# esologic/GANce

Measured on AMD Instinct MI355X. Metric: synthesized frames/sec at 1024x1024 config-f, higher is better.
Workload: dtype f32 (bf16x3 split operands, 6 terms, fp32 accumulate)

## Files before the change

### gance_amd/csrc/upfir_split.hip

```cpp

#include <hip/hip_runtime.h>

#include <algorithm>
#include <cstring>
#include <type_traits>

#include "kernels.h"

#ifndef GANCE_UPFIRS_ABLATE
#define GANCE_UPFIRS_ABLATE 0
#endif

namespace gance {

namespace {

typedef float f32x4 __attribute__((ext_vector_type(4)));
typedef float f32x2 __attribute__((ext_vector_type(2)));
typedef unsigned u32x4 __attribute__((ext_vector_type(4)));
typedef unsigned u32x2 __attribute__((ext_vector_type(2)));
typedef __bf16 bf16x8 __attribute__((ext_vector_type(8)));
typedef __bf16 bf16x2 __attribute__((ext_vector_type(2)));
typedef __attribute__((address_space(3))) void* lds_ptr_t;

constexpr int kBM = 16;
constexpr int kKC = 32;
constexpr int kSW = 64;
constexpr int kTH = 8;
constexpr int kRows = kTH + 1;
constexpr int kPlanes = 12;
constexpr int kPlaneStride = 80;
constexpr int kSlotUnits = kPlanes * kPlaneStride;
constexpr int kRing = 3;
constexpr int kHaloCols = 4;
constexpr int kHaloUnits = kRows * kHaloCols * kPlanes;
constexpr int kHaloTasks = kRows * kHaloCols * 4;
constexpr int kWeave = 2;
constexpr int kMinSegRows = 16;
constexpr int kDepth = 6;
constexpr int kCarryRows = 3;
constexpr int kPassCh = 4;
constexpr int kPassRows = 8;
constexpr float kSqrt2f = 1.4142135623730951f;
static_assert((2 * kRows) % kDepth == 0 && kDepth + 2 < kRows && kRows % kRing == 0, "ring slots and staging registers rotate with the unrolled rows of a chunk pair");

template <int NT>
struct Geo {
    static constexpr int kSW = 64 / NT;
    static constexpr int kBMB = kBM * NT;
    static constexpr int kTC = kSW / 16;
    static constexpr int kPW = 4 / NT;
    static constexpr int kTW = 2 * kSW + 4;
    static constexpr int kCG = kSW / 2;
    static constexpr int kRG = 64 / NT / kCG;
    static constexpr int kFR = kPassRows / kRG;
    static constexpr int kWin = kFR + 3;
    static constexpr int kCarryFloats = kBMB * kCarryRows * kTW;
    static constexpr int kStageFloats = kPassCh * NT * kPassRows * kTW;
    static constexpr int kNzPieces = 2 * kPassRows * 2 * kSW / 256;
    static constexpr int kWUnits = NT == 1 ? 27 * 64 : 0;
};

constexpr size_t kRingBytes = (size_t)kRing * kSlotUnits * 16;
constexpr size_t kHaloBytes = (size_t)2 * kHaloUnits * 16;
template <int NT>
constexpr size_t lds_bytes(int cin) {
    using G = Geo<NT>;
    return kRingBytes + kHaloBytes + (size_t)G::kWUnits * 16 +
           sizeof(float) * ((size_t)G::kStageFloats + G::kNzPieces * 256 + G::kCarryFloats + cin + 3 * G::kBMB);
}

__host__ __device__ constexpr int tap_cls(int t) { return t < 4 ? 0 : (t < 6 ? 1 : (t < 8 ? 2 : 3)); }
__host__ __device__ constexpr int tap_dy(int t) { return (t == 2 || t == 3 || t == 5) ? 1 : 0; }
__host__ __device__ constexpr int tap_dx(int t) { return (t == 1 || t == 3 || t == 7) ? 1 : 0; }

__device__ __forceinline__ void lds_barrier() {
    asm volatile("s_waitcnt lgkmcnt(0)" ::: "memory");
    __builtin_amdgcn_s_barrier();
    asm volatile("" ::: "memory");
}

__device__ __forceinline__ int fresh_lane() {
    int l;
    asm volatile("v_mbcnt_lo_u32_b32 %0, -1, 0\n\tv_mbcnt_hi_u32_b32 %0, -1, %0" : "=v"(l));
    return l;
}

__device__ __forceinline__ int ring_column(int P) {
    return ((P >> 2) & 3) | ((((P >> 4) ^ P) & 1) << 2) | (((P >> 1) & 1) << 3) | ((P & 1) << 4) | (P & 32);
}
constexpr int kEdgeColumn = 64;

__device__ __forceinline__ void split_pair(float a, float b, unsigned& p0, unsigned& p1, unsigned& p2) {
    auto pack = [](float lo, float hi) { return __builtin_bit_cast(unsigned, __builtin_convertvector(f32x2{lo, hi}, bf16x2)); };
    p0 = pack(a, b);
    const float ra = a - __builtin_bit_cast(float, p0 << 16), rb = b - __builtin_bit_cast(float, p0 & 0xffff0000u);
    p1 = pack(ra, rb);
    const float sa = ra - __builtin_bit_cast(float, p1 << 16), sb = rb - __builtin_bit_cast(float, p1 & 0xffff0000u);
    p2 = pack(sa, sb);
}

__device__ __forceinline__ void split_unit(const unsigned (&raw)[8], u32x4 (&part)[3]) {
    unsigned w[3][4];
    if (GANCE_UPFIRS_ABLATE & 1) {
#pragma unroll
        for (int q = 0; q < 3; ++q) part[q] = u32x4{raw[q], raw[q + 1], raw[q + 2], raw[q + 3]};
        return;
    }
#pragma unroll
    for (int e = 0; e < 4; ++e) split_pair(__builtin_bit_cast(float, raw[2 * e]), __builtin_bit_cast(float, raw[2 * e + 1]), w[0][e], w[1][e], w[2][e]);
#pragma unroll
    for (int q = 0; q < 3; ++q) part[q] = u32x4{w[q][0], w[q][1], w[q][2], w[q][3]};
}

}

template <int NT, bool kPre, bool kNoise>
__device__ __forceinline__ void upfirs_body(const UpFirArgs& p) {
    using G = Geo<NT>;
    constexpr int kSW = G::kSW, kBMB = G::kBMB, kTC = G::kTC, kPW = G::kPW, kTW = G::kTW, kCG = G::kCG, kRG = G::kRG, kFR = G::kFR,
                  kWin = G::kWin, kCarryFloats = G::kCarryFloats, kStageFloats = G::kStageFloats, kNzPieces = G::kNzPieces;
    extern __shared__ __attribute__((aligned(16))) unsigned char smem_raw[];
    u32x4* const ring = reinterpret_cast<u32x4*>(smem_raw);
    u32x4* const halo = ring + kRing * kSlotUnits;
    u32x4* const w_lds = halo + 2 * kHaloUnits;
    float* const stage = reinterpret_cast<float*>(w_lds + G::kWUnits);
    float* const nz_lds = stage + kStageFloats;
    float* const carry = nz_lds + kNzPieces * 256;
    float* const s_lds = carry + kCarryFloats;
    float* const d_lds = s_lds + (kPre ? 0 : p.Cin);
    float* const b_lds = d_lds + kBMB;
    float* const sn_lds = b_lds + kBMB;

    const int tid = threadIdx.x;
    const int wave = __builtin_amdgcn_readfirstlane(tid >> 6);
    const int lane = tid & 63;
    const int n16 = lane & 15, kg = lane >> 4;
    const int ct = NT == 1 ? 0 : wave / kTC, tc = NT == 1 ? wave : wave % kTC;

    int id;
    {
        const int v = blockIdx.x, nwg = p.total_blocks;
        const int q = nwg >> 3, r = nwg & 7, xcd = v & 7;
        id = (xcd < r ? xcd * (q + 1) : r * (q + 1) + (xcd - r) * q) + (v >> 3);
    }
    const int m_tile = id % p.m_tiles;
    id /= p.m_tiles;
    const int strip = id % p.strips;
    id /= p.strips;
    const int seg = id % p.segs;
    const int b = id / p.segs;
    const int m0 = m_tile * kBMB;
    const int X0 = strip * kSW;
    const int H = p.H, W = p.W;
    const int Hp = H + 2, Wp = W + 8;
    const int HpWp4 = Hp * Wp * 4;
    const int chunks = p.Cin / kKC;
    const int steps = H / kTH;
    const int s_begin = seg * (p.rows_per_seg / kTH), s_end = s_begin + p.rows_per_seg / kTH;
    const int s_first = seg > 0 ? s_begin - 1 : s_begin;

    const __amdgpu_buffer_rsrc_t x_rsrc =
        __builtin_amdgcn_make_buffer_rsrc((void*)(p.x + (size_t)b * p.x_b_stride), 0, p.Cin * Hp * Wp * 4, 0x00020000);
    const __amdgpu_buffer_rsrc_t w_rsrc = __builtin_amdgcn_make_buffer_rsrc(
        (void*)(reinterpret_cast<const unsigned char*>(p.w) + (size_t)(m_tile * NT + ct) * chunks * 27 * 1024), 0, chunks * 27 * 1024, 0x00020000);

    const int st_pair = lane >> 4, st_g = lane & 15;
    u32x4* const ring_w = ring + wave * kPlaneStride + ring_column(4 * st_g + st_pair);
    unsigned* const ring_wn = reinterpret_cast<unsigned*>(ring + wave * kPlaneStride + ring_column(NT == 2 ? 2 * st_g + (st_pair & 1) : st_g)) +
                              (NT == 2 ? 2 * (st_pair >> 1) : st_pair);
    const int m_pos = 16 * tc + n16;
    const u32x4* const ring_r0 = ring + kg * kPlaneStride + ring_column(m_pos);
    const u32x4* const ring_r1 = ring + kg * kPlaneStride + (m_pos > 0 ? ring_column(m_pos - 1) : kEdgeColumn);
    const bool edge_copy = wave == 3 && lane < kPlanes;
    const int e_unit = lane % kPlanes;
    u32x4* const ring_e = ring + (e_unit >> 2) * 4 * kPlaneStride + (e_unit & 3) * kPlaneStride + (edge_copy ? kEdgeColumn : 66 + wave);
    const u32x4* const halo_e = halo + e_unit;
    const u32x4* const halo_r = halo + ((n16 & 7) * kHaloCols + 2 * (n16 >> 3)) * kPlanes + kg;
    const u32x4* const halo_f = halo + ((kRows - 1) * kHaloCols + 2 * (n16 >> 3)) * kPlanes + kg;
    const int st_voff = (2 * st_pair * Hp * Wp + X0 + 4 + kPW * st_g) * 4;
    unsigned st[kDepth][8];
    auto stage_load = [&](unsigned(&dst)[8], int chunk, int brow, bool in_loop = false) {
        if ((GANCE_UPFIRS_ABLATE & 4) && in_loop) return;
        const int soff = ((chunk * kKC + wave * 8) * Hp + brow) * Wp * 4;
#pragma unroll
        for (int e = 0; e < 2; ++e) {
            if constexpr (kPW == 4) {
                const u32x4 q4 = __builtin_amdgcn_raw_buffer_load_b128(x_rsrc, st_voff, soff + e * HpWp4, 0);
#pragma unroll
                for (int c = 0; c < 4; ++c) dst[2 * c + e] = q4[c];
            } else if constexpr (kPW == 2) {
                const u32x2 q2 = __builtin_amdgcn_raw_buffer_load_b64(x_rsrc, st_voff, soff + e * HpWp4, 0);
                dst[e] = q2[0];
                dst[2 + e] = q2[1];
            } else {
                dst[e] = __builtin_amdgcn_raw_buffer_load_b32(x_rsrc, st_voff, soff + e * HpWp4, 0);
            }
        }
    };
    auto scale_pair = [&](unsigned(&raw)[8], int chunk) {
        if constexpr (!kPre) {
            const f32x2 s2 = *reinterpret_cast<const f32x2*>(s_lds + chunk * kKC + 8 * wave + 2 * st_pair);
#pragma unroll
            for (int c = 0; c < kPW; ++c) {
                raw[2 * c] = __builtin_bit_cast(unsigned, __builtin_bit_cast(float, raw[2 * c]) * s2[0]);
                raw[2 * c + 1] = __builtin_bit_cast(unsigned, __builtin_bit_cast(float, raw[2 * c + 1]) * s2[1]);
            }
        }
    };
    auto transpose_rows = [](u32x4& u) {
        auto a02 = __builtin_amdgcn_permlane32_swap(u[0], u[2], false, false);
        auto a13 = __builtin_amdgcn_permlane32_swap(u[1], u[3], false, false);
        auto b01 = __builtin_amdgcn_permlane16_swap(a02[0], a13[0], false, false);
        auto b23 = __builtin_amdgcn_permlane16_swap(a02[1], a13[1], false, false);
        u = u32x4{b01[0], b01[1], b23[0], b23[1]};
    };
    auto scale8 = [&](unsigned(&raw)[8], int chunk, int group) {
        if constexpr (!kPre) {
            const f32x4 s0 = *reinterpret_cast<const f32x4*>(s_lds + chunk * kKC + group * 8);
            const f32x4 s1 = *reinterpret_cast<const f32x4*>(s_lds + chunk * kKC + group * 8 + 4);
#pragma unroll
            for (int e = 0; e < 4; ++e) {
                raw[e] = __builtin_bit_cast(unsigned, __builtin_bit_cast(float, raw[e]) * s0[e]);
                raw[4 + e] = __builtin_bit_cast(unsigned, __builtin_bit_cast(float, raw[4 + e]) * s1[e]);
            }
        }
    };
    auto stage_store = [&](unsigned(&raw)[8], int slot, int chunk) {
        scale_pair(raw, chunk);
        if constexpr (NT == 1) {
            u32x4 part[3];
            split_unit(raw, part);
#pragma unroll
            for (int q = 0; q < 3; ++q) transpose_rows(part[q]);
#pragma unroll
            for (int q = 0; q < 3; ++q)
                if (!(GANCE_UPFIRS_ABLATE & 16)) ring_w[slot * kSlotUnits + q * 4 * kPlaneStride] = part[q];
        } else {
            unsigned w[3][kPW];
#pragma unroll
            for (int c = 0; c < kPW; ++c) split_pair(__builtin_bit_cast(float, raw[2 * c]), __builtin_bit_cast(float, raw[2 * c + 1]), w[0][c], w[1][c], w[2][c]);
#pragma unroll
            for (int q = 0; q < 3; ++q) {
                unsigned* const dst = ring_wn + 4 * (slot * kSlotUnits + q * 4 * kPlaneStride);
                if constexpr (NT == 2) {
                    const auto s = __builtin_amdgcn_permlane16_swap(w[q][0], w[q][1], false, false);
                    *reinterpret_cast<u32x2*>(dst) = u32x2{s[0], s[1]};
                } else {
                    *dst = w[q][0];
                }
            }
        }
    };
    auto edge_store = [&](int slot, int hbuf, int hrow) { if (!(GANCE_UPFIRS_ABLATE & 64)) ring_e[slot * kSlotUnits] = halo_e[hbuf * kHaloUnits + (hrow * kHaloCols + 1) * kPlanes]; };
    const int h_task = tid < kHaloTasks ? tid : tid - kHaloTasks;
    const int h_col = h_task & 3, h_kg = (h_task >> 2) & 3, h_row = h_task >> 4;
    const int h_voff = ((h_kg * 8 * Hp + h_row) * Wp + X0 + 2 + (h_col & 1) + (h_col >> 1) * (kSW + 1)) * 4;
    u32x4* const halo_w = halo + (h_row * kHaloCols + h_col) * kPlanes + h_kg;
    unsigned hraw[8];
    auto halo_load = [&](int step, int chunk) {
        const int soff = (chunk * kKC * Hp + kTH * step) * Wp * 4;
#pragma unroll
        for (int e = 0; e < 8; ++e) hraw[e] = __builtin_amdgcn_raw_buffer_load_b32(x_rsrc, h_voff, soff + e * HpWp4, 0);
    };
    auto halo_store = [&](int chunk, int buf) {
        scale8(hraw, chunk, h_kg);
        u32x4 part[3];
        split_unit(hraw, part);
#pragma unroll
        for (int q = 0; q < 3; ++q) halo_w[buf * kHaloUnits + q * 4] = part[q];
    };

    u32x4 A[9][3];
    const int a_voff = lane * 16;
    auto weights_dma = [&](int chunk) {
#pragma unroll
        for (int k = 0; k < 7; ++k)
            if (k < 6 || wave < 3)
                __builtin_amdgcn_raw_ptr_buffer_load_lds(w_rsrc, (lds_ptr_t)(w_lds + (wave + 4 * k) * 64), 16, lane * 16, (chunk * 27 + wave + 4 * k) * 1024, 0, 0);
    };
    const u32x4* const w_r = w_lds + lane;
    auto read_a3 = [&](int t, u32x4(&dst)[3]) {
#pragma unroll
        for (int q = 0; q < 3; ++q) dst[q] = w_r[(t * 3 + q) * 64];
    };
    auto load_a3 = [&](int chunk, int t, u32x4(&dst)[3]) {
#pragma unroll
        for (int q = 0; q < 3; ++q) dst[q] = __builtin_amdgcn_raw_buffer_load_b128(w_rsrc, a_voff, (chunk * 27 + t * 3 + q) * 1024, 0);
    };

    u32x4 Bf[2][2][3];
    auto load_b = [&](int slot, u32x4(&dst)[2][3]) {
#pragma unroll
        for (int q = 0; q < 3; ++q) {
            dst[0][q] = ring_r0[slot * kSlotUnits + q * 4 * kPlaneStride];
            dst[1][q] = ring_r1[slot * kSlotUnits + q * 4 * kPlaneStride];
        }
    };

    stage_load(st[0], 0, kTH * s_first + 0);
    stage_load(st[1], 0, kTH * s_first + 1);
    load_a3(0, 0, A[0]);
    halo_load(s_first, 0);
    if constexpr (!kPre)
        for (int i = tid; i < p.Cin; i += 256) s_lds[i] = p.s[(size_t)b * p.s_stride + i];
    if (tid < kBMB) {
        d_lds[tid] = p.d[(size_t)b * p.d_stride + m0 + tid];
        b_lds[tid] = p.bias[m0 + tid];
        sn_lds[tid] = p.s_next != nullptr ? p.s_next[(size_t)b * p.s_stride + m0 + tid] : 1.0f;
    }
    for (int i = tid; i < kCarryFloats; i += 256) carry[i] = 0.f;
    if constexpr (NT > 1)
        for (int i = tid; i < kPassCh * NT * kPassRows; i += 256) stage[i * kTW] = stage[i * kTW + 2 * kSW + 2] = stage[i * kTW + 2 * kSW + 3] = 0.f;
#pragma unroll
    for (int t = 1; t < 9; ++t) load_a3(0, t, A[t]);
    if constexpr (!kPre) lds_barrier();
    stage_store(st[0], 0, 0);
    stage_store(st[1], 1, 0);
    halo_store(0, 0);
#pragma unroll
    for (int r = 2; r < 2 + kDepth; ++r) stage_load(st[r % kDepth], 0, kTH * s_first + r);
    lds_barrier();
    edge_store(0, 0, 0);
    edge_store(1, 0, 1);
    lds_barrier();
    load_b(0, Bf[0]);

    const int OW = 2 * W, OWp = OW + 8;
    const long long oplane = (long long)(2 * H + 2) * OWp;
    const __amdgpu_buffer_rsrc_t o_rsrc = __builtin_amdgcn_make_buffer_rsrc(
        (void*)(p.out + ((size_t)b * p.Cout + m0) * oplane - 2 * OWp), 0, 0x7fffffff, 0x00020000);
    const __amdgpu_buffer_rsrc_t nz_rsrc = __builtin_amdgcn_make_buffer_rsrc(
        (void*)(kNoise ? p.noise + (size_t)b * p.noise_b_stride : nullptr), 0, kNoise ? (2 * H) * (2 * W) * 4 : 0, 0x00020000);
    const float ns2 = p.noise_strength * kSqrt2f;

    constexpr int kTerms[6][2] = {{2, 0}, {0, 2}, {1, 1}, {1, 0}, {0, 1}, {0, 0}};
    constexpr int kTapTurn[9] = {0, 4, 6, 8, 2, 5, 1, 7, 3};

#pragma unroll 1
    for (int si = s_first; si < s_end; ++si) {
        const int y0 = kTH * si;
        const bool last_step = si + 1 == steps;
        const bool priming = si < s_begin;
        f32x4 acc[kTH][4];
#pragma unroll
        for (int r = 0; r < kTH; ++r)
#pragma unroll
            for (int c = 0; c < 4; ++c) acc[r][c] = f32x4{0.f, 0.f, 0.f, 0.f};
        f32x4 accf[2] = {f32x4{0.f, 0.f, 0.f, 0.f}, f32x4{0.f, 0.f, 0.f, 0.f}};
        f32x4 acch[NT == 1 ? 1 : 2] = {}, acchf = f32x4{0.f, 0.f, 0.f, 0.f};

        auto run_chunk = [&](auto parity, const int chunk) {
            constexpr int ab = decltype(parity)::value;
            const int n_chunk = chunk + 1 < chunks ? chunk + 1 : 0;
            const int n_step = chunk + 1 < chunks ? si : (last_step ? si : si + 1);
#pragma unroll
            for (int j = 0; j < kRows; ++j) {
                const int cur = (j + ab) & 1;
                if (NT == 1 && j == 0) weights_dma(n_chunk);
                if (j == 0) halo_load(n_step, n_chunk);
                if (j == 4) halo_store(n_chunk, ab ^ 1);
                load_b((j + 1) % kRing, Bf[cur ^ 1]);
                edge_store((j + 2) % kRing, j + 2 < kRows ? ab : ab ^ 1, (j + 2) % kRows);
                stage_store(st[(kRows * ab + j + 2) % kDepth], (j + 2) % kRing, j + 2 < kRows ? chunk : n_chunk);
                stage_load(st[(kRows * ab + j + 2) % kDepth], j + 2 + kDepth < kRows ? chunk : n_chunk, kTH * (j + 2 + kDepth < kRows ? si : n_step) + (j + 2 + kDepth) % kRows, true);
                if (j + 1 < kRows) {
#pragma unroll
                    for (int term = 0; term < ((GANCE_UPFIRS_ABLATE & 8) ? 0 : 6); ++term)
#pragma unroll
                        for (int k = 0; k < 9; ++k) {
                            const int t = kTapTurn[k];
                            const int row = tap_dy(t) ? j : j - 1;
                            if (row < 0 || row >= kTH) continue;
                            acc[row][tap_cls(t)] = __builtin_amdgcn_mfma_f32_16x16x32_bf16(
                                __builtin_bit_cast(bf16x8, A[t][kTerms[term][1]]), __builtin_bit_cast(bf16x8, Bf[cur][tap_dx(t)][kTerms[term][0]]),
                                acc[row][tap_cls(t)], 0, 0, 0);
                        }
#pragma unroll
                    for (int i = 0; i < 54; ++i) {
                        if (i >= (j == 0 ? 18 : 54)) break;
                        __builtin_amdgcn_sched_group_barrier(0x008, 1, 0);
                        __builtin_amdgcn_sched_group_barrier(0x092, kWeave, 0);
                    }
                } else {
                    constexpr int kOrder[9] = {2, 3, 5, 0, 1, 4, 6, 7, 8};
#pragma unroll
                    for (int i = 0; i < 9; ++i) {
                        const int t = kOrder[i];
                        if (!tap_dy(t)) {
#pragma unroll
                            for (int term = 0; term < 6; ++term)
                                acc[kTH - 1][tap_cls(t)] = __builtin_amdgcn_mfma_f32_16x16x32_bf16(
                                    __builtin_bit_cast(bf16x8, A[t][kTerms[term][1]]), __builtin_bit_cast(bf16x8, Bf[cur][tap_dx(t)][kTerms[term][0]]),
                                    acc[kTH - 1][tap_cls(t)], 0, 0, 0);
                        } else if (last_step) {
#pragma unroll
                            for (int term = 0; term < 6; ++term)
                                accf[tap_cls(t)] = __builtin_amdgcn_mfma_f32_16x16x32_bf16(
                                    __builtin_bit_cast(bf16x8, A[t][kTerms[term][1]]), __builtin_bit_cast(bf16x8, Bf[cur][tap_dx(t)][kTerms[term][0]]),
                                    accf[tap_cls(t)], 0, 0, 0);
                        }
                        const int hc = NT == 1 ? 0 : tap_cls(t) >> 1;
                        const bool halo_mine = NT == 1 ? wave == tap_cls(t) : (tap_dx(t) && (tap_cls(t) & 1) == 0 && (kTC == 1 || tc == hc));
                        if (halo_mine && !(GANCE_UPFIRS_ABLATE & 64)) {
                            u32x4 hf[3];
#pragma unroll
                            for (int q = 0; q < 3; ++q) hf[q] = halo_r[ab * kHaloUnits + ((1 - tap_dy(t)) * kHaloCols + 1 - tap_dx(t)) * kPlanes + q * 4];
#pragma unroll
                            for (int term = 0; term < 6; ++term)
                                acch[hc] = __builtin_amdgcn_mfma_f32_16x16x32_bf16(__builtin_bit_cast(bf16x8, A[t][kTerms[term][1]]),
                                                                                    __builtin_bit_cast(bf16x8, hf[kTerms[term][0]]), acch[hc], 0, 0, 0);
                            if (last_step && tap_dy(t)) {
#pragma unroll
                                for (int q = 0; q < 3; ++q) hf[q] = halo_f[ab * kHaloUnits + (1 - tap_dx(t)) * kPlanes + q * 4];
#pragma unroll
                                for (int term = 0; term < 6; ++term)
                                    acchf = __builtin_amdgcn_mfma_f32_16x16x32_bf16(__builtin_bit_cast(bf16x8, A[t][kTerms[term][1]]),
                                                                                    __builtin_bit_cast(bf16x8, hf[kTerms[term][0]]), acchf, 0, 0, 0);
                            }
                        }
                        if constexpr (NT == 1) read_a3(t, A[t]);
                        else load_a3(n_chunk, t, A[t]);
                    }
                }
                if (NT == 1 && j == kRows - 2) asm volatile("s_waitcnt vmcnt(24)" ::: "memory");
                if (!(GANCE_UPFIRS_ABLATE & 32)) lds_barrier();
            }
        };
#pragma unroll 1
        for (int chunk = 0; chunk < chunks; chunk += 2) {
            run_chunk(std::integral_constant<int, 0>{}, chunk);
            run_chunk(std::integral_constant<int, 1>{}, chunk + 1);
        }

        const int elane = fresh_lane();
        const int en16 = elane & 15, eq4 = elane >> 4;
        const int dump_base = (4 * ct + eq4) * (kPassRows * kTW) + 32 * tc + 2 * en16 + 1;
        const int hpy = wave >> 1, hpx = wave & 1;
        const int fsub = NT == 1 ? 0 : elane / (64 / NT), flane = NT == 1 ? elane : elane % (64 / NT);
        const int fc = NT == 1 ? wave : wave * NT + fsub;
        const int fch = NT == 1 ? fc : 16 * (fc >> 2) + (fc & 3);
        const int cg = flane % kCG;
        const int rg = flane / kCG;
        const int o_voff = (int)((fch * oplane + (long long)(kFR * rg) * OWp + 4 * cg) * 4);

        auto run_passes = [&](auto flush_tag) {
            constexpr bool kFlush = decltype(flush_tag)::value;
            const int ys = kFlush ? H : y0;
            if (kNoise) {
#pragma unroll
                for (int i = 0; i < (kNzPieces + 3) / 4; ++i) {
                    if (kNzPieces % 4 != 0 && wave + 4 * i >= kNzPieces) break;
                    const int f = (wave + 4 * i) * 256 + 4 * elane;
                    const int row = f / (2 * kSW), col = f % (2 * kSW);
                    __builtin_amdgcn_raw_ptr_buffer_load_lds(nz_rsrc, (lds_ptr_t)(nz_lds + (wave + 4 * i) * 256), 16,
                                                             ((2 * ys - 2 + row) * OW + 2 * X0 + col) * 4, 0, 0, 0);
                }
                asm volatile("s_waitcnt vmcnt(0)" ::: "memory");
            }
            constexpr int kRowPasses = kFlush ? 1 : 2;
#pragma unroll
            for (int rw = 0; rw < kRowPasses; ++rw) {
                const int oy0 = 2 * (ys + 4 * rw) - 2;
                const int r_lo = max(0, -oy0);
                const int r_hi = priming ? 0 : min(kPassRows, 2 * H - oy0);
#pragma unroll
                for (int g = 0; g < 4; ++g) {
                    if constexpr (kFlush) {
#pragma unroll
                        for (int c = 0; c < 4; ++c) stage[dump_base + (c >> 1) * kTW + (c & 1)] = c < 2 ? accf[c][g] : 0.f;
                        if constexpr (NT == 1) {
                            if (en16 == 0 || en16 == 8) {
                                const int side = en16 >> 3;
                                if (hpy == 0 && (side == 1 || hpx == 1)) stage[eq4 * (kPassRows * kTW) + (side ? 2 * kSW + 1 + hpx : 0)] = acchf[g];
                                if (hpy == 1 && (side == 1 || hpx == 1)) stage[eq4 * (kPassRows * kTW) + kTW + (side ? 2 * kSW + 1 + hpx : 0)] = 0.f;
                            }
                        } else if (en16 == 8 && tc == 0) {
                            stage[(4 * ct + eq4) * (kPassRows * kTW) + 2 * kSW + 1] = acchf[g];
                            stage[(4 * ct + eq4) * (kPassRows * kTW) + kTW + 2 * kSW + 1] = 0.f;
                        }
                    } else {
#pragma unroll
                        for (int r4 = 0; r4 < 4; ++r4)
#pragma unroll
                            for (int c = 0; c < 4; ++c) stage[dump_base + (2 * r4 + (c >> 1)) * kTW + (c & 1)] = acc[4 * rw + r4][c][g];
                        const int row = en16 & 7, side = en16 >> 3;
                        if constexpr (NT == 1) {
                            if ((side == 1 || hpx == 1) && row / 4 == rw)
                                stage[eq4 * (kPassRows * kTW) + (2 * (row % 4) + hpy) * kTW + (side ? 2 * kSW + 1 + hpx : 0)] = acch[0][g];
                        } else if (side == 1 && row / 4 == rw) {
#pragma unroll
                            for (int h = 0; h < 2; ++h)
                                if (kTC == 1 || tc == h) stage[(4 * ct + eq4) * (kPassRows * kTW) + (2 * (row % 4) + h) * kTW + 2 * kSW + 1] = acch[h][g];
                        }
                    }
                    lds_barrier();

                    const int ch = 4 * g + fch;
                    const float dsc = d_lds[ch] * kSqrt2f;
                    const float kh0 = 0.25f * dsc, kh1 = 0.75f * dsc;
                    const float bias2 = b_lds[ch] * kSqrt2f;
                    const float lr6 = 0.6f * sn_lds[ch], lr4 = 0.4f * sn_lds[ch];
                    const float* const win_lo = carry + ch * (kCarryRows * kTW) + (kFR * rg) * kTW + 4 * cg;
                    const float* const win_hi = stage + fc * (kPassRows * kTW) + (kFR * rg - kCarryRows) * kTW + 4 * cg;
                    f32x4 ta[kWin], tb[kWin];
#pragma unroll
                    for (int i = 0; i < kWin; ++i) {
                        const float* const rowp = (i < kCarryRows && kFR * rg + i < kCarryRows ? win_lo : win_hi) + i * kTW;
                        ta[i] = *reinterpret_cast<const f32x4*>(rowp);
                        tb[i] = *reinterpret_cast<const f32x4*>(rowp + 4);
                    }
                    {
                        const int o_soff = (int)((4 * g * oplane + (long long)(oy0 + 3) * OWp + 2 * X0 + 4) * 4);
#pragma unroll
                        for (int r = 0; r < kFR; ++r) {
                            const int rr = kFR * rg + r;
                            if (rr >= r_lo && rr < r_hi) {
                                f32x2 tv[4];
#pragma unroll
                                for (int c2 = 0; c2 < 4; ++c2) {
                                    auto pair = [&](int i) { return c2 < 2 ? f32x2{ta[i][2 * c2], ta[i][2 * c2 + 1]} : f32x2{tb[i][2 * c2 - 4], tb[i][2 * c2 - 3]}; };
                                    tv[c2] = 0.25f * pair(r) + 0.75f * pair(r + 1) + 0.75f * pair(r + 2) + 0.25f * pair(r + 3);
                                }
                                const float t[7] = {tv[0][0], tv[0][1], tv[1][0], tv[1][1], tv[2][0], tv[2][1], tv[3][0]};
                                f32x4 v;
#pragma unroll
                                for (int o = 0; o < 4; ++o) v[o] = fmaf(kh0, t[o + 3], fmaf(kh1, t[o + 2], fmaf(kh1, t[o + 1], fmaf(kh0, t[o], bias2))));
                                if (kNoise) v += ns2 * *reinterpret_cast<const f32x4*>(nz_lds + (kPassRows * rw + rr) * (2 * kSW) + 4 * cg);
#pragma unroll
                                for (int o = 0; o < 4; ++o) v[o] = fmaf(lr6, v[o], lr4 * __builtin_fabsf(v[o]));
                                if (!(GANCE_UPFIRS_ABLATE & 128)) __builtin_amdgcn_raw_buffer_store_b128(__builtin_bit_cast(u32x4, v), o_rsrc, o_voff, o_soff + r * OWp * 4, 0);
                                else asm volatile("" ::"v"(v));
                            }
                        }
                    }
                    lds_barrier();
                    if (!kFlush && rg == kRG - 1) {
                        float* const carry_w = carry + ch * (kCarryRows * kTW) + 4 * cg;
#pragma unroll
                        for (int i = 0; i < 3; ++i) {
                            *reinterpret_cast<f32x4*>(carry_w + i * kTW) = ta[kWin - 3 + i];
                            if (cg == kCG - 1) *reinterpret_cast<f32x4*>(carry_w + i * kTW + 4) = tb[kWin - 3 + i];
                        }
                    }
                }
            }
        };
        if (GANCE_UPFIRS_ABLATE & 2) {
            float sum = acch[0][0] + acchf[0] + accf[0][0] + accf[1][0];
#pragma unroll
            for (int r = 0; r < kTH; ++r)
#pragma unroll
                for (int c = 0; c < 4; ++c) sum += acc[r][c][0] + acc[r][c][3];
            if (sum == 12345.678f) p.out[tid] = sum;
            continue;
        }
        run_passes(std::false_type{});
        if (last_step) {
            lds_barrier();
            run_passes(std::true_type{});
        }
    }
}

bool upfirs_supported(int cin, int cout, int H, int W) {
    return H == W && W % kSW == 0 && H % kTH == 0 && cin % (2 * kKC) == 0 && cout % kBM == 0 && cin <= 512;
}

bool upfirs_narrow_supported(int cin, int cout, int H, int W) {
    return H == W && (W == 32 || W == 16) && H % kTH == 0 && cin % (2 * kKC) == 0 && cout % (kBM * (kSW / W)) == 0 && cin <= 512;
}

size_t upfirs_weight_floats(int cin, int cout) { return (size_t)(cout / kBM) * (cin / kKC) * 27 * 256; }

static unsigned short bf16_rne_host(float x) {
    unsigned u;
    std::memcpy(&u, &x, 4);
    u += 0x7fffu + ((u >> 16) & 1u);
    return (unsigned short)(u >> 16);
}
static float bf16_value_host(unsigned short h) {
    const unsigned u = (unsigned)h << 16;
    float f;
    std::memcpy(&f, &u, 4);
    return f;
}

void upfirs_arrange_weights(const float* w_in, int cin, int cout, const int* up_tap_weight, float* w_out) {
    unsigned short* const out = reinterpret_cast<unsigned short*>(w_out);
    const int m_tiles = cout / kBM, chunks = cin / kKC;
    for (int mt = 0; mt < m_tiles; ++mt)
        for (int ch = 0; ch < chunks; ++ch)
            for (int t = 0; t < 9; ++t)
                for (int k = 0; k < kKC; ++k)
                    for (int m = 0; m < kBM; ++m) {
                        const int channel = 4 * (m & 3) + (m >> 2);
                        const float v = w_in[((size_t)up_tap_weight[t] * cin + ch * kKC + k) * cout + mt * kBM + channel];
                        unsigned short part[3];
                        part[0] = bf16_rne_host(v);
                        const float r1 = v - bf16_value_host(part[0]);
                        part[1] = bf16_rne_host(r1);
                        part[2] = bf16_rne_host(r1 - bf16_value_host(part[1]));
                        for (int q = 0; q < 3; ++q)
                            out[((((((size_t)mt * chunks + ch) * 9 + t) * 3 + q) * 4 + k / 8) * 16 + m) * 8 + k % 8] = part[q];
                    }
}

void upfirs_plan(int B, int cout, int H, int W, int num_cus, UpFirArgs* a) {
    a->step_rows = kTH;
    if (W < kSW) {
        a->m_tiles = cout / (kBM * (kSW / W));
        a->strips = 1;
        a->segs = 1;
        a->rows_per_seg = H;
        a->total_blocks = B * a->m_tiles;
        return;
    }
    a->m_tiles = cout / kBM;
    a->strips = W / kSW;
    int segs = 1;
    const int base = B * a->m_tiles * a->strips;
    long long best = (long long)((base + num_cus - 1) / num_cus) * H;
    for (int n = 2; H / n >= kMinSegRows && (H / n) % kTH == 0 && base * (n / 2) < num_cus; n *= 2) {
        const long long cost = (long long)((base * n + num_cus - 1) / num_cus) * (H / n + kTH);
        if (cost < best) best = cost, segs = n;
    }
    a->segs = segs;
    a->rows_per_seg = H / segs;
    a->total_blocks = base * segs;
}

__global__ __launch_bounds__(256, 1) void upfirs_fused_kernel(const UpFirArgs p) { upfirs_body<1, false, false>(p); }
__global__ __launch_bounds__(256, 1) void upfirs_fused_noise_kernel(const UpFirArgs p) { upfirs_body<1, false, true>(p); }
__global__ __launch_bounds__(256, 1) void upfirs_fused_pre_kernel(const UpFirArgs p) { upfirs_body<1, true, false>(p); }
__global__ __launch_bounds__(256, 1) void upfirs_fused_pre_noise_kernel(const UpFirArgs p) { upfirs_body<1, true, true>(p); }
__global__ __launch_bounds__(256, 1) void upfirs_w32_fused_kernel(const UpFirArgs p) { upfirs_body<2, false, false>(p); }
__global__ __launch_bounds__(256, 1) void upfirs_w32_fused_noise_kernel(const UpFirArgs p) { upfirs_body<2, false, true>(p); }
__global__ __launch_bounds__(256, 1) void upfirs_w32_fused_pre_kernel(const UpFirArgs p) { upfirs_body<2, true, false>(p); }
__global__ __launch_bounds__(256, 1) void upfirs_w32_fused_pre_noise_kernel(const UpFirArgs p) { upfirs_body<2, true, true>(p); }
__global__ __launch_bounds__(256, 1) void upfirs_w16_fused_kernel(const UpFirArgs p) { upfirs_body<4, false, false>(p); }
__global__ __launch_bounds__(256, 1) void upfirs_w16_fused_noise_kernel(const UpFirArgs p) { upfirs_body<4, false, true>(p); }
__global__ __launch_bounds__(256, 1) void upfirs_w16_fused_pre_kernel(const UpFirArgs p) { upfirs_body<4, true, false>(p); }
__global__ __launch_bounds__(256, 1) void upfirs_w16_fused_pre_noise_kernel(const UpFirArgs p) { upfirs_body<4, true, true>(p); }

hipError_t launch_upfir_split(const UpFirArgs& args, hipStream_t stream) {
    using Kernel = void (*)(const UpFirArgs);
    static const Kernel kernels[3][4] = {
        {upfirs_fused_kernel, upfirs_fused_noise_kernel, upfirs_fused_pre_kernel, upfirs_fused_pre_noise_kernel},
        {upfirs_w32_fused_kernel, upfirs_w32_fused_noise_kernel, upfirs_w32_fused_pre_kernel, upfirs_w32_fused_pre_noise_kernel},
        {upfirs_w16_fused_kernel, upfirs_w16_fused_noise_kernel, upfirs_w16_fused_pre_kernel, upfirs_w16_fused_pre_noise_kernel}};
    static size_t (*const lds_of[3])(int) = {lds_bytes<1>, lds_bytes<2>, lds_bytes<4>};
    static PerDeviceInt ready;
    int unused = 0;
    const hipError_t e = ready.get(
        [&](int, int* value) {
            *value = 1;
            for (int gi = 0; gi < 3; ++gi)
                for (int i = 0; i < 4; ++i) {
                    const hipError_t err = hipFuncSetAttribute(reinterpret_cast<const void*>(kernels[gi][i]), hipFuncAttributeMaxDynamicSharedMemorySize,
                                                               (int)lds_of[gi](i >= 2 ? 0 : 512));
                    if (err != hipSuccess) return err;
                }
            return hipSuccess;
        },
        &unused);
    if (e != hipSuccess) return e;
    const int gi = args.W % kSW == 0 ? 0 : (args.W == 32 ? 1 : 2);
    const bool narrow = gi != 0;
    if (!(narrow ? upfirs_narrow_supported(args.Cin, args.Cout, args.H, args.W) : upfirs_supported(args.Cin, args.Cout, args.H, args.W)) || args.segs < 1 ||
        args.rows_per_seg * args.segs != args.H || args.rows_per_seg % kTH != 0 || args.total_blocks != args.B * args.m_tiles * args.strips * args.segs ||
        (narrow && (args.segs != 1 || args.strips != 1 || args.m_tiles * kBM * (kSW / args.W) != args.Cout)))
        return hipErrorInvalidValue;
    const int pre = args.input_prescaled ? 1 : 0, noise = args.noise != nullptr ? 1 : 0;
    hipLaunchKernelGGL(kernels[gi][2 * pre + noise], dim3(args.total_blocks), dim3(256), lds_of[gi](pre ? 0 : args.Cin), stream, args);
    return hipGetLastError();
}

}
```

Measured before the change: 1496.

## Grow LDS ring to four slots and barrier every two rows

Enlarges the LDS staging ring from three to four slots, split into two halves that swap once per chunk pair. With the extra slot, staging stores run three rows ahead instead of two, and the workgroup barrier fires only on odd rows, roughly halving the barrier count in the main loop. The vmcnt waits are re-tuned for the new prefetch distance. The cost is more LDS per block, which may reduce occupancy, plus more complex slot indexing that risks subtle race bugs.

```diff
diff --git a/gance_amd/csrc/upfir_split.hip b/gance_amd/csrc/upfir_split.hip
--- a/gance_amd/csrc/upfir_split.hip
+++ b/gance_amd/csrc/upfir_split.hip
@@ -31,7 +31,7 @@
 constexpr int kPlanes = 12;
 constexpr int kPlaneStride = 80;
 constexpr int kSlotUnits = kPlanes * kPlaneStride;
-constexpr int kRing = 3;
+constexpr int kRing = 4;
 constexpr int kHaloCols = 4;
 constexpr int kHaloUnits = kRows * kHaloCols * kPlanes;
 constexpr int kHaloTasks = kRows * kHaloCols * 4;
@@ -42,7 +42,8 @@
 constexpr int kPassCh = 4;
 constexpr int kPassRows = 8;
 constexpr float kSqrt2f = 1.4142135623730951f;
-static_assert((2 * kRows) % kDepth == 0 && kDepth + 2 < kRows && kRows % kRing == 0, "ring slots and staging registers rotate with the unrolled rows of a chunk pair");
+static_assert(kRing == 4 && (2 * kRows) % 2 == 0 && (2 * kRows) % kRing == 2, "barrier intervals of two rows; the ring halves change places once per chunk pair");
+static_assert((2 * kRows) % kDepth == 0 && kDepth + 3 <= kRows, "the staging registers rotate with the unrolled rows of a chunk pair");
 
 template <int NT>
 struct Geo {
@@ -69,6 +70,8 @@
     return kRingBytes + kHaloBytes + (size_t)G::kWUnits * 16 +
            sizeof(float) * ((size_t)G::kStageFloats + G::kNzPieces * 256 + G::kCarryFloats + cin + 3 * G::kBMB);
 }
+
+static_assert(lds_bytes<1>(512) <= 160 * 1024 && lds_bytes<2>(512) <= 160 * 1024 && lds_bytes<4>(512) <= 160 * 1024, "a block's LDS is the CU's 160 KB at most");
 
 __host__ __device__ constexpr int tap_cls(int t) { return t < 4 ? 0 : (t < 6 ? 1 : (t < 8 ? 2 : 3)); }
 __host__ __device__ constexpr int tap_dy(int t) { return (t == 2 || t == 3 || t == 5) ? 1 : 0; }
@@ -165,6 +168,10 @@
     const __amdgpu_buffer_rsrc_t w_rsrc = __builtin_amdgcn_make_buffer_rsrc(
         (void*)(reinterpret_cast<const unsigned char*>(p.w) + (size_t)(m_tile * NT + ct) * chunks * 27 * 1024), 0, chunks * 27 * 1024, 0x00020000);
 
+    constexpr int kHalfUnits = 2 * kSlotUnits;
+    int half0 = 0;
+    auto swap_halves = [&] { half0 = kHalfUnits - half0; };
+    auto slot_of = [&](int r) { return (((r >> 1) & 1) ? kHalfUnits - half0 : half0) + (r & 1) * kSlotUnits; };
     const int st_pair = lane >> 4, st_g = lane & 15;
     u32x4* const ring_w = ring + wave * kPlaneStride + ring_column(4 * st_g + st_pair);
     unsigned* const ring_wn = reinterpret_cast<unsigned*>(ring + wave * kPlaneStride + ring_column(NT == 2 ? 2 * st_g + (st_pair & 1) : st_g)) +
@@ -226,7 +233,7 @@
             }
         }
     };
-    auto stage_store = [&](unsigned(&raw)[8], int slot, int chunk) {
+    auto stage_store = [&](unsigned(&raw)[8], int r, int chunk) {
         scale_pair(raw, chunk);
         if constexpr (NT == 1) {
             u32x4 part[3];
@@ -235,14 +242,14 @@
             for (int q = 0; q < 3; ++q) transpose_rows(part[q]);
 #pragma unroll
             for (int q = 0; q < 3; ++q)
-                if (!(GANCE_UPFIRS_ABLATE & 16)) ring_w[slot * kSlotUnits + q * 4 * kPlaneStride] = part[q];
+                if (!(GANCE_UPFIRS_ABLATE & 16)) ring_w[slot_of(r) + q * 4 * kPlaneStride] = part[q];
         } else {
             unsigned w[3][kPW];
 #pragma unroll
             for (int c = 0; c < kPW; ++c) split_pair(__builtin_bit_cast(float, raw[2 * c]), __builtin_bit_cast(float, raw[2 * c + 1]), w[0][c], w[1][c], w[2][c]);
 #pragma unroll
             for (int q = 0; q < 3; ++q) {
-                unsigned* const dst = ring_wn + 4 * (slot * kSlotUnits + q * 4 * kPlaneStride);
+                unsigned* const dst = ring_wn + 4 * (slot_of(r) + q * 4 * kPlaneStride);
                 if constexpr (NT == 2) {
                     const auto s = __builtin_amdgcn_permlane16_swap(w[q][0], w[q][1], false, false);
                     *reinterpret_cast<u32x2*>(dst) = u32x2{s[0], s[1]};
@@ -252,7 +259,7 @@
             }
         }
     };
-    auto edge_store = [&](int slot, int hbuf, int hrow) { if (!(GANCE_UPFIRS_ABLATE & 64)) ring_e[slot * kSlotUnits] = halo_e[hbuf * kHaloUnits + (hrow * kHaloCols + 1) * kPlanes]; };
+    auto edge_store = [&](int r, int hbuf, int hrow) { if (!(GANCE_UPFIRS_ABLATE & 64)) ring_e[slot_of(r)] = halo_e[hbuf * kHaloUnits + (hrow * kHaloCols + 1) * kPlanes]; };
     const int h_task = tid < kHaloTasks ? tid : tid - kHaloTasks;
     const int h_col = h_task & 3, h_kg = (h_task >> 2) & 3, h_row = h_task >> 4;
     const int h_voff = ((h_kg * 8 * Hp + h_row) * Wp + X0 + 2 + (h_col & 1) + (h_col >> 1) * (kSW + 1)) * 4;
@@ -290,16 +297,17 @@
     };
 
     u32x4 Bf[2][2][3];
-    auto load_b = [&](int slot, u32x4(&dst)[2][3]) {
+    auto load_b = [&](int r, u32x4(&dst)[2][3]) {
 #pragma unroll
         for (int q = 0; q < 3; ++q) {
-            dst[0][q] = ring_r0[slot * kSlotUnits + q * 4 * kPlaneStride];
-            dst[1][q] = ring_r1[slot * kSlotUnits + q * 4 * kPlaneStride];
+            dst[0][q] = ring_r0[slot_of(r) + q * 4 * kPlaneStride];
+            dst[1][q] = ring_r1[slot_of(r) + q * 4 * kPlaneStride];
         }
     };
 
     stage_load(st[0], 0, kTH * s_first + 0);
     stage_load(st[1], 0, kTH * s_first + 1);
+    stage_load(st[2], 0, kTH * s_first + 2);
     load_a3(0, 0, A[0]);
     halo_load(s_first, 0);
     if constexpr (!kPre)
@@ -317,12 +325,14 @@
     if constexpr (!kPre) lds_barrier();
     stage_store(st[0], 0, 0);
     stage_store(st[1], 1, 0);
+    stage_store(st[2], 2, 0);
     halo_store(0, 0);
 #pragma unroll
-    for (int r = 2; r < 2 + kDepth; ++r) stage_load(st[r % kDepth], 0, kTH * s_first + r);
+    for (int r = 3; r < 3 + kDepth; ++r) stage_load(st[r % kDepth], 0, kTH * s_first + r);
     lds_barrier();
     edge_store(0, 0, 0);
     edge_store(1, 0, 1);
+    edge_store(2, 0, 2);
     lds_barrier();
     load_b(0, Bf[0]);
 
@@ -356,14 +366,15 @@
             const int n_step = chunk + 1 < chunks ? si : (last_step ? si : si + 1);
 #pragma unroll
             for (int j = 0; j < kRows; ++j) {
-                const int cur = (j + ab) & 1;
-                if (NT == 1 && j == 0) weights_dma(n_chunk);
+                const int r = kRows * ab + j;
+                const int cur = r & 1;
+                if (NT == 1 && j == ab) weights_dma(n_chunk);
                 if (j == 0) halo_load(n_step, n_chunk);
                 if (j == 4) halo_store(n_chunk, ab ^ 1);
-                load_b((j + 1) % kRing, Bf[cur ^ 1]);
-                edge_store((j + 2) % kRing, j + 2 < kRows ? ab : ab ^ 1, (j + 2) % kRows);
-                stage_store(st[(kRows * ab + j + 2) % kDepth], (j + 2) % kRing, j + 2 < kRows ? chunk : n_chunk);
-                stage_load(st[(kRows * ab + j + 2) % kDepth], j + 2 + kDepth < kRows ? chunk : n_chunk, kTH * (j + 2 + kDepth < kRows ? si : n_step) + (j + 2 + kDepth) % kRows, true);
+                load_b(r + 1, Bf[cur ^ 1]);
+                edge_store(r + 3, j + 3 < kRows ? ab : ab ^ 1, (j + 3) % kRows);
+                stage_store(st[(r + 3) % kDepth], r + 3, j + 3 < kRows ? chunk : n_chunk);
+                stage_load(st[(r + 3) % kDepth], n_chunk, kTH * n_step + j, true);
                 if (j + 1 < kRows) {
 #pragma unroll
                     for (int term = 0; term < ((GANCE_UPFIRS_ABLATE & 8) ? 0 : 6); ++term)
@@ -423,14 +434,20 @@
                         else load_a3(n_chunk, t, A[t]);
                     }
                 }
-                if (NT == 1 && j == kRows - 2) asm volatile("s_waitcnt vmcnt(24)" ::: "memory");
-                if (!(GANCE_UPFIRS_ABLATE & 32)) lds_barrier();
+                if (NT == 1 && ab == 0 && j == kRows - 2) asm volatile("s_waitcnt vmcnt(24)" ::: "memory");
+                if (NT == 1 && ab == 1 && j == kRows - 3) asm volatile("s_waitcnt vmcnt(12)" ::: "memory");
+                if (r & 1) {
+                    if (!(GANCE_UPFIRS_ABLATE & 32)) lds_barrier();
+                } else if (j == kRows - 1) {
+                    __builtin_amdgcn_sched_barrier(0);
+                }
             }
         };
 #pragma unroll 1
         for (int chunk = 0; chunk < chunks; chunk += 2) {
             run_chunk(std::integral_constant<int, 0>{}, chunk);
             run_chunk(std::integral_constant<int, 1>{}, chunk + 1);
+            swap_halves();
         }
 
         const int elane = fresh_lane();
```

Measured after the change: 1496. No clear change (-0.0%).
